# achinastone/Tensorium

Hardware: AMD Instinct MI355X
Metric: fp32 SGEMM GFLOP/s (M=N=K=4096) + YOLOv3 conv-fwd images/s (higher is better)
Workload: dtype fp32; 1 GPU; sgemm_nn_4096x4096x4096; M=4096, N=4096, K=4096, parallelism=1 independent replicas, one process per GPU, no data-path collective

## Files before the change

### tensorium_amd/csrc/sgemm_nn_big.hip

```cpp
#include <type_traits>

#include "tns_internal.hpp"

namespace tns {
namespace {

typedef float floatx16 __attribute__((ext_vector_type(16)));

template <int BM, int BN, int WM, int WN, int MINB, int BK = 32>
struct Geo {
  static constexpr int BM_ = BM, BN_ = BN, WN_ = WN, MINB_ = MINB, BK_ = BK;
  static constexpr int KQ = BK / 4;
  static constexpr int NT = 64 * WM * WN;
  static constexpr int WTM = BM / WM, WTN = BN / WN;
  static constexpr int TM = WTM / 32, TN = WTN / 32;
  static constexpr int LDA = BM, LDB = BN;
  static constexpr int A_TILE = BK * LDA, B_TILE = BK * LDB;
  static constexpr int STAGE = A_TILE + B_TILE;
  static constexpr int AU = BM * BK / 4 / NT;
  static constexpr int BROWS = 256 / BN;
  static constexpr int BDMA = BK / BROWS / (NT / 64);
  static_assert(TM == 2 || TM == 4, "A fragments read as one b64 / b128");
  static_assert(BN == 128 || BN == 256, "B rows of 512 B or 1 KB per DMA");
  static_assert(AU >= 1 && BDMA >= 1 && BM * BK / 4 % NT == 0, "staging split");
  static_assert(BK == 16 || BK == 32, "k-quad swizzle over at most 8 quads");
};

template <class G>
__global__ __launch_bounds__(G::NT, G::MINB_) void sgemm_nn_big_kernel(GemmArgs p) {
  constexpr int BM = G::BM_, BN = G::BN_, NT = G::NT, WN = G::WN_;
  constexpr int WTM = G::WTM, WTN = G::WTN, TM = G::TM, TN = G::TN;
  constexpr int LDA = G::LDA, LDB = G::LDB, A_TILE = G::A_TILE, STAGE = G::STAGE;
  constexpr int AU = G::AU, BK = G::BK_, KQ = G::KQ;
  constexpr int SW = KQ == 8 ? 2 : 4;
  const int tid = threadIdx.x, lane = tid & 63, wid = tid >> 6;
  const int lc = lane & 31, h = lane >> 5;
  const int wm = wid / WN, wn = wid % WN;
  __shared__ __attribute__((aligned(16))) float smem[2 * STAGE];

  const int tiles_m = (int)(p.M / BM), tiles_n = (int)(p.N / BN);
  int tm, tn;
  {
    const int nb = tiles_m * tiles_n, bid = blockIdx.x;
    const int xcd = bid & 7, q = nb >> 3, r = nb & 7;
    const int wg = (xcd < r ? xcd * (q + 1) : r * (q + 1) + (xcd - r) * q) + (bid >> 3);
    constexpr int GROUP_M = 8;
    const int per_group = GROUP_M * tiles_n;
    const int group = wg / per_group, first_m = group * GROUP_M;
    const int gsize = min(tiles_m - first_m, GROUP_M);
    const int in_group = wg - group * per_group;
    tm = first_m + in_group % gsize;
    tn = in_group / gsize;
  }
  const int64_t m0 = (int64_t)tm * BM, n0 = (int64_t)tn * BN, bz = blockIdx.y;
  const float* __restrict__ A = p.A + bz * p.strideA;
  const float* __restrict__ B = p.B + bz * p.strideB;
  float* __restrict__ C = p.C + bz * p.strideC;
  const int64_t lda = p.lda, ldb = p.ldb, ldc = p.ldc;

  floatx16 acc[TM][TN];
  const int64_t row_base = m0 + wm * WTM + 4 * h;
  const int64_t col_base = n0 + wn * WTN + lc;
  if (p.beta_mode == BETA_ZERO) {
#pragma unroll
    for (int i = 0; i < TM; ++i)
#pragma unroll
      for (int j = 0; j < TN; ++j)
#pragma unroll
        for (int e = 0; e < 16; ++e) acc[i][j][e] = 0.0f;
  } else {
    const bool scale = p.beta_mode == BETA_SCALE;
    const float beta = p.beta;
#pragma unroll
    for (int i = 0; i < TM; ++i)
#pragma unroll
      for (int j = 0; j < TN; ++j)
#pragma unroll
        for (int e = 0; e < 16; ++e)
          acc[i][j][e] = C[(row_base + 32 * i + (e & 3) + 8 * (e >> 2)) * ldc + col_base + 32 * j];
    if (scale) {
#pragma unroll
      for (int i = 0; i < TM; ++i)
#pragma unroll
        for (int j = 0; j < TN; ++j)
#pragma unroll
          for (int e = 0; e < 16; ++e) acc[i][j][e] = beta * acc[i][j][e];
    }
  }
#pragma unroll
  for (int i = 0; i < TM; ++i)
#pragma unroll
    for (int j = 0; j < TN; ++j) asm volatile("" : "+v"(acc[i][j]));

  const float* a_src[AU];
  int a_dst[AU];
#pragma unroll
  for (int u = 0; u < AU; ++u) {
    const int idx = tid + NT * u;
    const int kq = idx % KQ, mm = idx / KQ;
    const int m = (mm & ~(WTM - 1)) | ((mm % TM) << 5) | ((mm & (WTM - 1)) / TM);
    a_src[u] = A + (m0 + m) * lda + 4 * kq;
    a_dst[u] = (4 * kq) * LDA + (mm ^ (kq << SW));
  }
  float4 ra[AU];
  const float alpha = p.alpha;
  auto load_a = [&](int64_t k0) {
#pragma unroll
    for (int u = 0; u < AU; ++u) ra[u] = *reinterpret_cast<const float4*>(a_src[u] + k0);
  };
  auto store_a = [&](float* as) {
#pragma unroll
    for (int u = 0; u < AU; ++u) {
      float4 v = ra[u];
      v.x = alpha * v.x; v.y = alpha * v.y; v.z = alpha * v.z; v.w = alpha * v.w;
      as[a_dst[u]] = v.x;
      as[a_dst[u] + LDA] = v.y;
      as[a_dst[u] + 2 * LDA] = v.z;
      as[a_dst[u] + 3 * LDA] = v.w;
    }
  };
  constexpr int BROWS = G::BROWS, BDMA = G::BDMA;
  const int brow = BROWS * BDMA * wid + lane / (BN / 4);
  const float* b_src = B + (int64_t)brow * ldb + n0 + 4 * (lane % (BN / 4));
  const unsigned b_lds0 = __builtin_amdgcn_readfirstlane(
      (unsigned)(uintptr_t)(__attribute__((address_space(3))) float*)(smem + A_TILE +
                                                                      BROWS * BDMA * wid * LDB));
  auto dma_b = [&](int64_t k0, int stage) {
#pragma unroll
    for (int r = 0; r < BDMA; ++r) {
      unsigned keep;
      const float* src = b_src + (k0 + BROWS * r) * ldb;
      asm volatile(
          "s_mov_b32 %0, m0\n\ts_mov_b32 m0, %2\n\ts_nop 0\n\t"
          "global_load_lds_dwordx4 %1, off\n\ts_mov_b32 m0, %0"
          : "=&s"(keep)
          : "v"(src), "s"(b_lds0 + (unsigned)((stage * STAGE + BROWS * r * LDB) * 4))
          : "memory");
    }
  };

  const int a_frag = wm * WTM + TM * lc;
  const int b_frag = wn * WTN + lc;
  auto frag = [&](const float* st, int s, float (&a)[TM], float (&b)[TN]) {
    const int k = 2 * s + h;
#ifdef TNS_NB_NO_FRAG
    for (int i = 0; i < TM; ++i) a[i] = (float)(lane + i + s);
    for (int j = 0; j < TN; ++j) b[j] = (float)(lane - j + s);
    (void)st; (void)k;
    return;
#endif
    const float* ap = st + k * LDA + (a_frag ^ (((k >> 2) & (KQ - 1)) << SW));
    if constexpr (TM == 4) {
      const float4 v = *reinterpret_cast<const float4*>(ap);
      a[0] = v.x; a[1] = v.y; a[2] = v.z; a[3] = v.w;
    } else {
      const float2 v = *reinterpret_cast<const float2*>(ap);
      a[0] = v.x; a[1] = v.y;
    }
    const float* bp = st + A_TILE + k * LDB + b_frag;
#pragma unroll
    for (int j = 0; j < TN; ++j) b[j] = bp[32 * j];
  };
  auto mma = [&](const float (&a)[TM], const float (&b)[TN]) {
#pragma unroll
    for (int i = 0; i < TM; ++i)
#pragma unroll
      for (int j = 0; j < TN; ++j)
        acc[i][j] = __builtin_amdgcn_mfma_f32_32x32x2f32(a[i], b[j], acc[i][j], 0, 0, 0);
  };

  const int nt = (int)(p.K / BK);
  if (nt > 0) {
    load_a(0);
    dma_b(0, 0);
    store_a(smem);
    asm volatile("s_waitcnt vmcnt(0)" ::: "memory");
    __syncthreads();
  }
  auto tile = [&](int t, auto MORE) {
    constexpr bool more = decltype(MORE)::value;
    const float* cur = smem + (t & 1) * STAGE;
    float* nxt = smem + ((t + 1) & 1) * STAGE;
    if constexpr (more) {
#ifndef TNS_NB_NO_DMA
      dma_b((int64_t)(t + 1) * BK, (t + 1) & 1);
#endif
#ifndef TNS_NB_NO_AST
      load_a((int64_t)(t + 1) * BK);
#endif
      __builtin_amdgcn_sched_barrier(0);
    }
    float a0[TM], b0[TN], a1[TM], b1[TN];
    frag(cur, 0, a0, b0);
#pragma unroll
    for (int s = 0; s < BK / 2; s += 2) {
      frag(cur, s + 1, a1, b1);
      __builtin_amdgcn_sched_barrier(0);
      mma(a0, b0);
      if (s + 2 < BK / 2) frag(cur, s + 2, a0, b0);
      __builtin_amdgcn_sched_barrier(0);
      if constexpr (more)
        if (s == BK / 4 - 2) {
          __builtin_amdgcn_sched_barrier(0);
#ifndef TNS_NB_NO_AST
          store_a(nxt);
#endif
        }
      mma(a1, b1);
    }
    if constexpr (more) {
#ifndef TNS_NB_NO_BAR
      asm volatile("s_waitcnt vmcnt(0)" ::: "memory");
      __syncthreads();
#endif
    }
  };
  for (int t = 0; t + 1 < nt; ++t) tile(t, std::true_type{});
  if (nt > 0) tile(nt - 1, std::false_type{});

#pragma unroll
  for (int i = 0; i < TM; ++i)
#pragma unroll
    for (int e = 0; e < 16; ++e) {
      const int64_t row = row_base + 32 * i + (e & 3) + 8 * (e >> 2);
#pragma unroll
      for (int j = 0; j < TN; ++j) C[row * ldc + col_base + 32 * j] = acc[i][j][e];
    }
}

bool aligned16(const void* p) { return (reinterpret_cast<uintptr_t>(p) & 15) == 0; }

using G256 = Geo<256, 256, 2, 4, 1>;
using G128 = Geo<128, 128, 2, 2, 2>;
using G256x128 = Geo<256, 128, 2, 2, 1>;
using G256w16 = Geo<256, 256, 4, 4, 1>;
using G256x128k16 = Geo<256, 128, 2, 2, 2, 16>;

template <class G>
bool applies(const GemmArgs& a) {
  if (a.conv || a.epi != EPI_NONE || a.beta_mode == BETA_STORE) return false;
  if (a.M % G::BM_ || a.N % G::BN_ || a.K % G::BK_ || a.M <= 0 || a.N <= 0) return false;
  if (a.lda % 4 || a.ldb % 4 || !aligned16(a.A) || !aligned16(a.B)) return false;
  if (a.batch > 1 && (a.strideA % 4 || a.strideB % 4)) return false;
  return (a.M / G::BM_) * (a.N / G::BN_) <= 0x7fffffff;
}

template <class G>
hipError_t launch(const GemmArgs& a, hipStream_t s) {
  if (!applies<G>(a)) return hipErrorInvalidValue;
  const int64_t tiles = (a.M / G::BM_) * (a.N / G::BN_);
  for (int64_t b0 = 0; b0 < a.batch; b0 += 65535) {
    GemmArgs sub = a;
    const int64_t nb = a.batch - b0 < 65535 ? a.batch - b0 : 65535;
    sub.A = a.A + b0 * a.strideA;
    sub.B = a.B + b0 * a.strideB;
    sub.C = a.C + b0 * a.strideC;
    sub.batch = nb;
    hipLaunchKernelGGL(sgemm_nn_big_kernel<G>, dim3((unsigned)tiles, (unsigned)nb), dim3(G::NT), 0,
                       s, sub);
    hipError_t e = hipGetLastError();
    if (e != hipSuccess) return e;
  }
  return hipSuccess;
}

}

#ifdef TNS_DIAG_KERNELS
int sgemm_nn_big_count() { return 8; }
#else
int sgemm_nn_big_count() { return 7; }
#endif
const char* sgemm_nn_big_name(int v) {
  static const char* names[] = {"256x256x32_w2x4_nn_big", "128x128x32_w2x2_nn_big",
                                "256x128x32_w2x2_nn_big", "256x256x32_w4x4_nn_big",
                                "256x128x16_w2x2_b2_nn_big", "256x256x32_w2x4_pp_nn_big",
                                "256x256x32_w2x2_dma_nn_big", "256x256x32_w2x4_ppbq_nn_big"};
  return v >= 0 && v < sgemm_nn_big_count() ? names[v] : "";
}

int sgemm_nn_big_pick(const GemmArgs& a) {
  if (applies<G256>(a) && (a.M / 256) * (a.N / 256) * a.batch >= 192)
    return sgemm_nn_w4_applies(a) ? 6 : sgemm_nn_pp_applies(a) ? 5 : 0;
  return -1;
}

hipError_t launch_sgemm_nn_big(int v, const GemmArgs& a, hipStream_t s) {
  switch (v) {
    case 0: return launch<G256>(a, s);
    case 1: return launch<G128>(a, s);
    case 2: return launch<G256x128>(a, s);
    case 3: return launch<G256w16>(a, s);
    case 4: return launch<G256x128k16>(a, s);
    case 5: return launch_sgemm_nn_pp(a, s);
    case 6: return launch_sgemm_nn_w4(a, s);
#ifdef TNS_DIAG_KERNELS
    case 7: return launch_sgemm_nn_pp(a, s, true);
#endif
    default: return hipErrorInvalidValue;
  }
}

}
```

### tensorium_amd/csrc/sgemm_nn_w4.hip

```cpp
#include "tns_internal.hpp"

namespace tns {
namespace {

typedef float floatx16 __attribute__((ext_vector_type(16)));
typedef float floatx4 __attribute__((ext_vector_type(4)));
typedef int int4v __attribute__((ext_vector_type(4)));

constexpr int BM = 256, BN = 256, BK = 32, NT = 256;
constexpr int A_TILE = BM * BK, B_TILE = BK * BN, STAGE = A_TILE + B_TILE;

__device__ __forceinline__ void dma16(const float* sbase, unsigned voff, unsigned lds) {
  unsigned keep;
  asm volatile(
      "s_mov_b32 %0, m0\n\ts_mov_b32 m0, %3\n\ts_nop 0\n\t"
      "global_load_lds_dwordx4 %1, %2\n\ts_mov_b32 m0, %0"
      : "=&s"(keep)
      : "v"(voff), "s"(sbase), "s"(lds)
      : "memory");
}

template <bool ALPHA1>
__global__ __launch_bounds__(NT, 1) void sgemm_nn_w4_kernel(GemmArgs p) {
  __shared__ __attribute__((aligned(16))) float smem[2 * STAGE];
  const int tid = threadIdx.x, lane = tid & 63;
  const int wid = __builtin_amdgcn_readfirstlane(tid >> 6);
  const int lc = lane & 31, h = lane >> 5;
  const int wm = wid >> 1, wn = wid & 1;

  const int tiles_m = (int)(p.M / BM), tiles_n = (int)(p.N / BN);
  int tm, tn;
  const int64_t bz = blockIdx.y;
  {
    const int nb = tiles_m * tiles_n, bid = blockIdx.x;
    const int xcd = bid & 7, q = nb >> 3, r = nb & 7;
    const int wg = (xcd < r ? xcd * (q + 1) : r * (q + 1) + (xcd - r) * q) + (bid >> 3);
    constexpr int GROUP_M = 8;
    const int per_group = GROUP_M * tiles_n;
    const int group = wg / per_group, first_m = group * GROUP_M;
    const int gsize = min(tiles_m - first_m, GROUP_M);
    const int in_group = wg - group * per_group;
    tm = first_m + in_group % gsize;
    tn = in_group / gsize;
  }
  const int64_t m0 = (int64_t)tm * BM, n0 = (int64_t)tn * BN;
  const float* __restrict__ A = p.A + bz * p.strideA;
  const float* __restrict__ B = p.B + bz * p.strideB;
  float* __restrict__ C = p.C + bz * p.strideC;
  const int64_t lda = p.lda, ldb = p.ldb, ldc = p.ldc;

  const int arow = lane >> 3;
  const unsigned a_voff = (unsigned)(arow * lda * 4) + 16u * (unsigned)((lane & 7) ^ ((arow >> 1) & 7));
  const unsigned a_voff1 = (unsigned)(arow * lda * 4) +
                           16u * (unsigned)((lane & 7) ^ (((arow >> 1) & 7) ^ 4));
  const unsigned b_voff0 = 16u * (unsigned)lane;
  const unsigned b_voff1 = 16u * (unsigned)((lane + 8) & 63);
  const unsigned lds0 = (unsigned)(uintptr_t)(__attribute__((address_space(3))) float*)smem;
  const float* a_row0 = A + m0 * lda;
  const float* b_row0 = B + n0;
  auto issue1 = [&](int u, int64_t k0, int st) {
    const unsigned sb = lds0 + (unsigned)(st * STAGE * 4);
    if (u < 8) {
      const int q = 8 * wid + u;
      dma16(a_row0 + (int64_t)(8 * q) * lda + k0, (u & 1) ? a_voff1 : a_voff,
            sb + (unsigned)(q * 1024));
    } else {
      const int r = 8 * wid + (u - 8);
      dma16(b_row0 + (k0 + r) * ldb, (u & 1) ? b_voff1 : b_voff0,
            sb + (unsigned)(A_TILE * 4 + r * 1024));
    }
  };
  auto issue = [&](int64_t k0, int st) {
    const unsigned sb = lds0 + (unsigned)(st * STAGE * 4);
#pragma unroll
    for (int u = 0; u < 8; ++u) {
      const int q = 8 * wid + u;
      dma16(a_row0 + (int64_t)(8 * q) * lda + k0, (u & 1) ? a_voff1 : a_voff,
            sb + (unsigned)(q * 1024));
    }
#pragma unroll
    for (int u = 0; u < 8; ++u) {
      const int r = 8 * wid + u;
      dma16(b_row0 + (k0 + r) * ldb, (u & 1) ? b_voff1 : b_voff0,
            sb + (unsigned)(A_TILE * 4 + r * 1024));
    }
  };

  const int nt = (int)(p.K / BK);
#ifdef TNS_W4_DMA_LATE
  constexpr bool kDmaFirst = false;
#else
  constexpr bool kDmaFirst = true;
#endif
  if (kDmaFirst && nt > 0) issue(0, 0);
  if (kDmaFirst && nt > 1) issue(BK, 1);

  floatx16 acc[4][4];
  const int64_t row_base = m0 + wm * 128;
  const __amdgpu_buffer_rsrc_t crs = __builtin_amdgcn_make_buffer_rsrc(
      C + row_base * ldc, 0, 0x7fffffff, 0x00020000);
  const unsigned c_voff = 4u * (unsigned)(4 * h * ldc + n0 + wn * 128 + 4 * lc);
  auto c_soff = [&](int i, int e) {
    return (unsigned)(4 * (32 * i + (e & 3) + 8 * (e >> 2)) * ldc);
  };
  if (p.beta_mode == BETA_ZERO) {
#pragma unroll
    for (int i = 0; i < 4; ++i)
#pragma unroll
      for (int j = 0; j < 4; ++j)
#pragma unroll
        for (int e = 0; e < 16; ++e) acc[i][j][e] = 0.0f;
  } else {
    const bool scale = p.beta_mode == BETA_SCALE;
    const float beta = p.beta;
    {
      floatx4 v[2][4];
      auto ldv = [&](int g, floatx4 (&t)[4]) {
#pragma unroll
        for (int u = 0; u < 4; ++u)
          t[u] = __builtin_bit_cast(floatx4, __builtin_amdgcn_raw_buffer_load_b128(
                                                 crs, c_voff, c_soff(g >> 2, 4 * (g & 3) + u), 0));
      };
      ldv(0, v[0]);
#pragma unroll
      for (int g = 0; g < 16; ++g) {
        if (g + 1 < 16) ldv(g + 1, v[(g + 1) & 1]);
#pragma unroll
        for (int u = 0; u < 4; ++u)
#pragma unroll
          for (int j = 0; j < 4; ++j) {
            const float c = v[g & 1][u][j];
            acc[g >> 2][j][4 * (g & 3) + u] = scale ? beta * c : c;
          }
      }
    }
  }
#pragma unroll
  for (int i = 0; i < 4; ++i)
#pragma unroll
    for (int j = 0; j < 4; ++j) asm volatile("" : "+a"(acc[i][j]));
  if (!kDmaFirst && nt > 0) issue(0, 0);
  if (!kDmaFirst && nt > 1) issue(BK, 1);

  const int swz = (lc >> 1) & 7;
  int b_col[4];
#pragma unroll
  for (int j = 0; j < 4; ++j)
    b_col[j] = A_TILE + h * BN + ((wn * 128 + 4 * lc + j - 32 * h) & 255);
  const float alpha = p.alpha;
  auto mma = [&](const float (&a)[4], const float (&b)[4]) {
    float aa[4];
#pragma unroll
    for (int i = 0; i < 4; ++i) aa[i] = ALPHA1 ? a[i] : alpha * a[i];
#pragma unroll
    for (int i = 0; i < 4; ++i)
#pragma unroll
      for (int j = 0; j < 4; ++j)
        acc[i][j] = __builtin_amdgcn_mfma_f32_32x32x2f32(aa[i], b[j], acc[i][j], 0, 0, 0);
  };
  auto mma_dma = [&](const float (&a)[4], const float (&b)[4], int64_t k0, int st, bool dma) {
    float aa[4];
#pragma unroll
    for (int i = 0; i < 4; ++i) aa[i] = ALPHA1 ? a[i] : alpha * a[i];
#pragma unroll
    for (int u = 0; u < 16; ++u) {
      const int i = u >> 2, j = u & 3;
      acc[i][j] = __builtin_amdgcn_mfma_f32_32x32x2f32(aa[i], b[j], acc[i][j], 0, 0, 0);
      if (dma) issue1(u, k0, st);
      __builtin_amdgcn_sched_barrier(0);
    }
  };

  const int a_lane = (wm * 128 + lc) * BK + h;
  auto frag = [&](const float* st, int s, float (&a)[4], float (&b)[4]) {
    const int ka = 4 * ((s >> 1) ^ swz) + 2 * (s & 1);
#pragma unroll
    for (int i = 0; i < 4; ++i) a[i] = st[a_lane + 32 * BK * i + ka];
    const floatx4 v = *reinterpret_cast<const floatx4*>(st + b_col[0] + 2 * s * BN);
    b[0] = v[0]; b[1] = v[1]; b[2] = v[2]; b[3] = v[3];
  };
  float a0[4], b0[4], a1[4], b1[4];
  {
    if (nt > 0) {
      if (nt > 1) {
        asm volatile("s_waitcnt vmcnt(16)" ::: "memory");
      } else {
        asm volatile("s_waitcnt vmcnt(0)" ::: "memory");
      }
      __syncthreads();
      frag(smem, 0, a0, b0);
    }
    for (int t = 0; t < nt; ++t) {
      const float* cur = smem + (t & 1) * STAGE;
      const float* nxt = smem + ((t + 1) & 1) * STAGE;
#pragma unroll
      for (int s = 0; s < BK / 2 - 2; s += 2) {
        frag(cur, s + 1, a1, b1);
        __builtin_amdgcn_sched_barrier(0);
        mma(a0, b0);
        frag(cur, s + 2, a0, b0);
        __builtin_amdgcn_sched_barrier(0);
        mma(a1, b1);
      }
      frag(cur, BK / 2 - 1, a1, b1);
      __builtin_amdgcn_sched_barrier(0);
      mma(a0, b0);
      __builtin_amdgcn_sched_barrier(0);
      if (t + 1 < nt) {
        asm volatile("s_waitcnt vmcnt(0)" ::: "memory");
        __syncthreads();
        frag(nxt, 0, a0, b0);
        __builtin_amdgcn_sched_barrier(0);
      }
      mma_dma(a1, b1, (int64_t)(t + 2) * BK, t & 1, t + 2 < nt);
    }
  }

#pragma unroll
  for (int i = 0; i < 4; ++i)
#pragma unroll
    for (int e = 0; e < 16; ++e) {
      const floatx4 v = {acc[i][0][e], acc[i][1][e], acc[i][2][e], acc[i][3][e]};
      __builtin_amdgcn_raw_buffer_store_b128(__builtin_bit_cast(int4v, v), crs, c_voff,
                                             c_soff(i, e), 0);
    }
}

bool aligned16(const void* q) { return (reinterpret_cast<uintptr_t>(q) & 15) == 0; }

}

bool sgemm_nn_w4_applies(const GemmArgs& a) {
  if (a.conv || a.epi != EPI_NONE || a.beta_mode == BETA_STORE) return false;
  if (a.M % BM || a.N % BN || a.K % BK || a.M <= 0 || a.N <= 0) return false;
  if (a.lda % 4 || a.ldb % 4 || !aligned16(a.A) || !aligned16(a.B)) return false;
  if (a.batch > 1 && (a.strideA % 4 || a.strideB % 4)) return false;
  if (a.lda * 4 * 8 > 0x7fffffffLL || (256 * a.ldc + a.N) * 4 > 0x7fffffffLL) return false;
  return (a.M / BM) * (a.N / BN) <= 0x7fffffff;
}

hipError_t launch_sgemm_nn_w4(const GemmArgs& a, hipStream_t s) {
  if (!sgemm_nn_w4_applies(a)) return hipErrorInvalidValue;
  const int64_t tiles = (a.M / BM) * (a.N / BN);
  const bool alpha1 = a.alpha == 1.0f;
  for (int64_t b0 = 0; b0 < a.batch; b0 += 65535) {
    GemmArgs sub = a;
    const int64_t nb = a.batch - b0 < 65535 ? a.batch - b0 : 65535;
    sub.A = a.A + b0 * a.strideA;
    sub.B = a.B + b0 * a.strideB;
    sub.C = a.C + b0 * a.strideC;
    sub.batch = nb;
    const dim3 grid((unsigned)tiles, (unsigned)nb);
    if (alpha1)
      hipLaunchKernelGGL((sgemm_nn_w4_kernel<true>), grid, dim3(NT), 0, s, sub);
    else
      hipLaunchKernelGGL((sgemm_nn_w4_kernel<false>), grid, dim3(NT), 0, s, sub);
    hipError_t e = hipGetLastError();
    if (e != hipSuccess) return e;
  }
  return hipSuccess;
}

}
```

### tensorium_amd/csrc/tns_internal.hpp

```cpp
#pragma once
#include <hip/hip_runtime.h>
#include <stdint.h>

#include "../../include/tns.h"

namespace tns {

int set_error(int code, const char* fmt, ...);
const char* hip_err_str(hipError_t e);

#define TNS_HIP_TRY(expr)                                                              \
  do {                                                                                 \
    hipError_t _e = (expr);                                                            \
    if (_e != hipSuccess)                                                              \
      return ::tns::set_error(TNS_ERR_HIP, "%s failed: %s (%s:%d)", #expr,            \
                              ::tns::hip_err_str(_e), __FILE__, __LINE__);             \
  } while (0)

enum EpiKind { EPI_NONE = 0, EPI_BIAS_ACT = 1, EPI_ADD = 2 };
constexpr bool act_transcendental(int act) { return act == 0 || act == 6; }

enum BetaMode { BETA_ZERO = 0, BETA_ONE = 1, BETA_SCALE = 2, BETA_STORE = 3 };

struct GemmArgs {
  int64_t M, N, K;
  float alpha, beta;
  int beta_mode;
  const float* A;
  int64_t lda, strideA;
  const float* B;
  int64_t ldb, strideB;
  float* C;
  int64_t ldc, strideC;
  int64_t batch;
  int epi;
  const float* bias;
  int act;
  int conv;
  const int* ktab;
  int ktab_n;
  int conv_H, conv_W, conv_ow, conv_ohw, conv_sY, conv_sX, conv_pH, conv_pW;
  int conv_bytes;
  int dx_cls, dx_taps, dx_imgW;
  unsigned* stamps;
};

hipError_t launch_sgemm(const GemmArgs& a, bool transA, bool transB, hipStream_t s);
int sgemm_nn_big_count();
const char* sgemm_nn_big_name(int v);
int sgemm_nn_big_pick(const GemmArgs& a);
hipError_t launch_sgemm_nn_big(int v, const GemmArgs& a, hipStream_t s);
bool sgemm_nn_pp_applies(const GemmArgs& a);
hipError_t launch_sgemm_nn_pp(const GemmArgs& a, hipStream_t s, bool bperm = false);
bool sgemm_nn_w4_applies(const GemmArgs& a);
hipError_t launch_sgemm_nn_w4(const GemmArgs& a, hipStream_t s);
hipError_t launch_sgemm_nt_sdot(const GemmArgs& a, hipStream_t s);
hipError_t launch_sdot_chains(const GemmArgs& a, int variant, hipStream_t s);
int sdot_chains_variant_count();
const char* sdot_chains_variant_name(int v);
int sdot_rc_variant_count();
const char* sdot_rc_variant_name(int v);
bool sdot_rc_applies(const GemmArgs& a);
hipError_t launch_sdot_rc(int v, const GemmArgs& a, hipStream_t s);
constexpr int SDOT_FORM_RC = 64;
void set_sdot_form(int form);
hipError_t launch_sgemm_tt(const GemmArgs& a, hipStream_t s);
hipError_t launch_add_in_order(float* C, const float* part, int64_t n, int64_t batch,
                               hipStream_t s);
hipError_t launch_sgemm_conv(const GemmArgs& a, hipStream_t s);
hipError_t launch_sgemm_conv_variant(int variant, const GemmArgs& a, hipStream_t s);
int conv_tile_count();
const char* conv_tile_name(int v);
int conv_tile_pick(const GemmArgs& a, int ks);
hipError_t launch_conv_tile(int v, const GemmArgs& a, int ks, int dil, hipStream_t s);
struct ConvSlabArgs {
  const float* input;
  const float* weights;
  const float* bias;
  float* out;
  int64_t batch, C, H, W, M, K, ks, stride, pad, dil, ow, ohw;
  int act;
};
int conv1x1_count();
const char* conv1x1_name(int v);
int conv1x1_pick(int64_t M, int64_t N, int64_t K, int64_t P);
hipError_t launch_conv1x1(int v, const float* weights, const float* x, const float* bias,
                          float* out, int64_t batch, int64_t M, int64_t K, int64_t P, int act,
                          hipStream_t s, bool add = false);
hipError_t launch_transpose(const float* in, float* out, int64_t rows, int64_t cols,
                            hipStream_t s);
int conv_slab_count();
const char* conv_slab_name(int v);
int conv_slab_pick(int64_t M, int64_t N, int64_t K, int64_t ks);
int64_t conv_slab_floats(int v, int64_t N, int64_t K);
hipError_t launch_conv_slab(int v, const ConvSlabArgs& c, float* slab, hipStream_t s);
int conv_tile4_count();
bool conv_tile4_is_ap(int v);
bool conv_tile_is_ap(int v);
hipError_t conv_tile4_permute(const float* A, float* Ap, int64_t M, int64_t K, hipStream_t s);
const char* conv_tile4_name(int v);
int conv_tile4_bk(int v);
hipError_t launch_conv_tile4(int v, const GemmArgs& a, int ks, int dil, hipStream_t s);
int conv_tile4_ta_count();
const char* conv_tile4_ta_name(int v);
int conv_tile4_dx_pick(int64_t M, int64_t N, int64_t K, int64_t ks);
hipError_t launch_conv_tile4_dx(int v, const float* w, const float* delta, float* col,
                                int64_t batch, int64_t C, int64_t ks, int64_t F, int64_t oh,
                                int64_t ow, hipStream_t s, bool add_into = false);
int conv_tile4_dx3_count();
const char* conv_tile4_dx3_name(int v);
int conv_tile4_dx3_pick(int64_t batch, int64_t C, int64_t H, int64_t W, int64_t F, int64_t ks,
                        int64_t pad);
hipError_t launch_conv_tile4_dx3(int v, const float* wt, const float* delta, float* im,
                                 int64_t batch, int64_t C, int64_t H, int64_t W, int64_t F,
                                 int64_t ks, int64_t pad, int64_t oh, int64_t ow, hipStream_t s);
hipError_t launch_transpose_taps(const float* w, float* wt, int64_t F, int64_t C, int64_t K2,
                                 hipStream_t s, unsigned long long order = ~0ULL);
unsigned long long conv_tile4_dx3s2_order(int64_t pad);
int conv_tile4_dx3s2_pick(int64_t batch, int64_t C, int64_t H, int64_t W, int64_t F, int64_t ks,
                          int64_t pad);
hipError_t launch_conv_tile4_dx3s2(int v, const float* wt, const float* delta, float* im,
                                   int64_t batch, int64_t C, int64_t H, int64_t W, int64_t F,
                                   int64_t pad, int64_t oh, int64_t ow, hipStream_t s);
int conv_pp_count();
const char* conv_pp_name(int v);
int conv_pp_pick(const GemmArgs& a, int ks);
hipError_t launch_conv_pp(int v, const GemmArgs& a, int ks, int dil, hipStream_t s);
int conv_dma_count();
const char* conv_dma_name(int v);
int conv_dma_pick(const GemmArgs& a, int ks);
hipError_t launch_conv_dma(int v, const GemmArgs& a, int ks, int dil, hipStream_t s);
int conv_patch_count();
const char* conv_patch_name(int v);
int conv_patch_pick(const GemmArgs& a);
hipError_t launch_conv_patch(int v, const GemmArgs& a, hipStream_t s);
struct DwArgs {
  const float* delta;
  const float* x;
  float* part;
  int M, N, HW, C, H, W, oW, stride, pad, dil;
  int va;
  float alpha;
  int64_t strideA, strideX, strideP, batch;
};
int dw_tile_count();
const char* dw_tile_name(int v);
int dw_tile_pick(const DwArgs& a, int ks);
hipError_t launch_dw_tile(int v, const DwArgs& a, int ks, hipStream_t s);
bool conv_direct_applies(int64_t C, int64_t ks, int64_t filters);
hipError_t launch_conv_direct(const float* in, const float* w, const float* bias, float* out,
                              int64_t batch, int64_t C, int64_t H, int64_t W, int64_t filters,
                              int64_t ks, int64_t stride, int64_t pad, int64_t dil, int64_t oh,
                              int64_t ow, int act, hipStream_t s);
bool conv_dx_fused_applies(int64_t C, int64_t H, int64_t W, int64_t ks, int64_t stride, int64_t F,
                           int64_t oh, int64_t ow);
bool conv_dx_fused_fits(int64_t C, int64_t H, int64_t W, int64_t stride, int64_t F, int64_t oh,
                        int64_t ow);
hipError_t launch_conv_dx_col2im(const float* w, float* wt, const float* delta, float* im,
                                 int64_t batch, int64_t C, int64_t H, int64_t W, int64_t F,
                                 int64_t ks, int64_t pad, int64_t dil, int64_t oh, int64_t ow,
                                 hipStream_t s);
constexpr int KTAB_PAD = 256;
hipError_t launch_build_ktab(int* ktab, int C, int Hs, int Ws, int kH, int kW, int dY, int dX,
                             hipStream_t s);
hipError_t launch_pad_images(const float* im, int64_t batch, int64_t C, int64_t H, int64_t W,
                             int64_t pH, int64_t pW, float* out, hipStream_t s);
hipError_t launch_sgemm_variant(int variant, const GemmArgs& a, bool transA, bool transB,
                                hipStream_t s);
int sgemm_variant_count();
const char* sgemm_variant_name(int v);

struct ConvGeom {
  int64_t C, H, W, kH, kW, padH, padW, sY, sX, dY, dX;
  int64_t oh, ow;
};
int64_t out_dim(int64_t in, int64_t pad, int64_t k, int64_t dil, int64_t stride);
hipError_t launch_im2col(const ConvGeom& g, const float* im, int64_t imStride, float* col,
                         int64_t colStride, int64_t batch, hipStream_t s);
hipError_t launch_col2im(const ConvGeom& g, const float* col, int64_t colStride, float* im,
                         int64_t imStride, int64_t batch, hipStream_t s);
struct DwResArgs {
  ConvGeom g;
  const float* x;
  int64_t xStride;
  const float* delta;
  float* weight_updates;
  float *dA, *dB, *part;
  int64_t M, N, K, batch;
  bool direct;
  float alpha;
};
int dw_res_count();
const char* dw_res_name(int v);
int64_t dw_res_k4(int64_t K);
int64_t dw_res_groups(int v);
int64_t dw_res_b_rows(int v, int64_t N);
int dw_res_pick(int64_t M, int64_t N, int64_t K, int64_t batch);
hipError_t launch_dw_res(int v, const DwResArgs& d, hipStream_t s);

bool act_supported(int act);
hipError_t launch_forward_bias(float* dst, int64_t nFilters, int64_t blockSize,
                               const float* bias, int64_t incb, int64_t batch, hipStream_t s);
hipError_t launch_backward_bias(float* dst, int64_t nDst, const float* src, int64_t blockSize,
                                int64_t batch, int64_t incb, hipStream_t s);
hipError_t launch_activate(float* x, int64_t n, int act, hipStream_t s);
hipError_t launch_shortcut(int64_t n, const float* a, const float* b, float* out, int act,
                           hipStream_t s);
hipError_t launch_upsample(int64_t planes, int H, int W, int stride, float scale, const float* in,
                           float* out, hipStream_t s);
hipError_t launch_upsample_backward(int64_t planes, int H, int W, int stride, float scale,
                                   float* in, const float* out, int zero, hipStream_t s);
struct PoolGeom {
  int h, w, outH, outW, size, sx, sy, off;
};
hipError_t launch_maxpool_forward(int64_t planes, const PoolGeom& g, const float* in, float* out,
                                  int64_t* indexes, hipStream_t s);
hipError_t launch_avgpool_forward(int64_t planes, const PoolGeom& g, const float* in, float* out,
                                  hipStream_t s);
hipError_t launch_maxpool_backward(int64_t planes, const PoolGeom& g, float* state_delta,
                                   const int64_t* indexes, const float* delta, hipStream_t s);
hipError_t launch_avgpool_backward(int64_t planes, const PoolGeom& g, float* state_delta,
                                   const float* delta, hipStream_t s);
hipError_t launch_dropout_forward(int64_t n, uint32_t seed, float probability, float scale,
                                  const float* src, float* rnd, float* dst, hipStream_t s);
hipError_t launch_dropout_backward(int64_t n, float probability, float scale, const float* src,
                                   const float* rnd, float* dst, hipStream_t s);
hipError_t launch_cost_l2(int64_t n, const float* pred, const float* truth, float* delta,
                          float* error, hipStream_t s);
hipError_t launch_xent_logistic(int64_t n, const float* pred, const float* truth, float* delta,
                                float* error, hipStream_t s);
hipError_t launch_lstm_gates_forward(int64_t n, const float* const w[4], const float* const u[4],
                                     float* c_state, float* h_state, float* cell_slice,
                                     float* out_slice, hipStream_t s);
hipError_t launch_lstm_gates_backward(int64_t n, const float* const w[4], const float* const u[4],
                                      const float* cell_i, const float* cprev,
                                      const float* delta_i, float* dc, float* const dw[4],
                                      float* const du[4], hipStream_t s);
hipError_t launch_vv(int op, int64_t n, const float* a, int64_t inca, const float* b, int64_t incb,
                     const float* c, int64_t incc, float* d, int64_t incd, hipStream_t s);
hipError_t launch_fmavss(int64_t n, const float* src, float scalar, float bias, float* dst,
                         hipStream_t s);
hipError_t launch_inverse_sqrt(int64_t n, const float* src, float* dst, int64_t stride,
                               hipStream_t s);
hipError_t launch_yolo(int64_t batch, int anchors, int classes, int64_t hw, const float* in,
                       float* out, hipStream_t s);
hipError_t launch_bias_activate(float* dst, int64_t nFilters, int64_t blockSize,
                                const float* bias, int64_t batch, int act, hipStream_t s);
hipError_t launch_derive(const float* x, int64_t n, int act, float* delta, hipStream_t s);
hipError_t launch_sgd_update(int64_t nw, float* w, float* dw, int64_t n, float* b, float* db,
                             float* sc, float* dsc, float lrb, float ndb, float mom,
                             hipStream_t s);
hipError_t launch_axpy(int64_t n, float a, const float* x, int64_t incx, float* y, int64_t incy,
                       hipStream_t s);
hipError_t launch_scale(int64_t n, float a, float* x, int64_t stride, hipStream_t s);
hipError_t launch_fill(int64_t n, float* x, float v, int64_t stride, hipStream_t s);
hipError_t launch_copy(int64_t n, const float* src, int64_t inca, float* dst, int64_t incb,
                       hipStream_t s);
hipError_t launch_clamp(int64_t n, float alpha, const float* src, float* dst, int64_t stride,
                        hipStream_t s);

hipError_t launch_means_vars(const float* x, int64_t groups, int64_t N, int64_t bs, float* means,
                             float* vars, int quirk, float* part, hipStream_t s, int what = 3);
hipError_t launch_normalize(float* x, int64_t groups, int64_t N, int64_t bs, const float* means,
                            int64_t mstride, const float* vars, int64_t vstride, hipStream_t s);
hipError_t launch_scale_add(float* x, int64_t groups, int64_t N, int64_t bs, const float* scales,
                            const float* biases, int64_t incb, hipStream_t s);
hipError_t launch_add_dots(float* dst, const float* a, const float* b, int64_t groups, int64_t N,
                           int64_t bs, float* part, hipStream_t s);
hipError_t launch_add_sums(float* dst, const float* src, int64_t groups, int64_t N, int64_t bs,
                           float* part, hipStream_t s);
hipError_t launch_derive_add_sums(float* dst, float* delta, const float* output, int act,
                                  int64_t groups, int64_t N, int64_t bs, float* part,
                                  hipStream_t s);
hipError_t launch_mean_var_delta(const float* delta, const float* x, const float* mean,
                                 const float* var, int64_t groups, int64_t N, int64_t bs,
                                 float* mean_delta, float* var_delta, int quirk, float* part,
                                 hipStream_t s, const float* scales = nullptr);
hipError_t launch_normalize_delta(const float* x, const float* mean, const float* var,
                                  const float* mean_delta, const float* var_delta, float* delta,
                                  int64_t groups, int64_t N, int64_t bs, hipStream_t s, const float* scales = nullptr); 
bool bn_folds_scale(int64_t bs);
hipError_t launch_bn_backward_fused(float* scale_updates, const float* x_norm, float* delta,
                                    const float* output, int act, const float* x,
                                    const float* mean, const float* var, const float* scales,
                                    float* mean_delta, float* var_delta, int64_t groups,
                                    int64_t N, int64_t bs, int quirk, float* part, hipStream_t s);
hipError_t launch_add_dots_derive(float* dst, const float* x_norm, float* delta,
                                  const float* output, int act, int64_t groups, int64_t N,
                                  int64_t bs, float* part, hipStream_t s);
hipError_t launch_bn_apply(const float* y, float* x, float* xn, float* out, int64_t groups,
                           int64_t N, int64_t bs, const float* means, const float* vars,
                           const float* scales, const float* biases, int act, hipStream_t s);
hipError_t launch_rolling_update(int64_t n, float* rm, float* rv, const float* mean,
                                 const float* var, float momentum, hipStream_t s);
hipError_t launch_softmax_batch(int64_t n, const float* in, int64_t batch, int64_t batch_size,
                                int64_t groups, int64_t group_size, int64_t stride, float temp,
                                float* out, hipStream_t s);
hipError_t launch_xent_softmax(int64_t n, const float* pred, const float* truth, float* delta,
                               float* error, hipStream_t s);
hipError_t launch_vssum(int64_t n, const float* a, float* out, hipStream_t s);

constexpr int MLP_MAX_LAYERS = 16;
struct MlpArgs {
  int nlayers;
  int64_t widths[MLP_MAX_LAYERS + 1];
  int acts[MLP_MAX_LAYERS];
  int bn;
  int64_t batch;
  const float* X;
  const float* truth;
  float lr, momentum, decay;
  float* buf;
  float* cost;
  int64_t off[MLP_MAX_LAYERS][16];
  int64_t softmax_off;
  int64_t stamp_off;
  int lds_chunks;
  int64_t act_off;
  float* l0part;
};
int64_t mlp_buffer_floats(int nlayers, const int64_t* widths, int bn, int64_t batch);
hipError_t launch_mlp_train_step(const MlpArgs& a, hipStream_t s);

}
```

Before: 143,900 GFLOP/s.

## Add row-wise prologue/epilogue to w4 SGEMM overlapping C load/store with MFMA

Adds a ROWS variant of the w4 kernel, the new default, that splits the prologue and epilogue into per-accumulator-row units. It streams C loads (beta path) and C stores row by row underneath the first and last K tiles' MFMAs instead of doing them all before or after the main loop. The aim is to hide the C read and write latency at the tile boundaries. It adds considerable code complexity, hand-written inline asm buffer loads, and a new dependence on correct waitcnt accounting.

Measured after the change: 146,500 GFLOP/s, median of 6. 1.8% higher.

```diff
diff --git a/tensorium_amd/csrc/sgemm_nn_big.hip b/tensorium_amd/csrc/sgemm_nn_big.hip
--- a/tensorium_amd/csrc/sgemm_nn_big.hip
+++ b/tensorium_amd/csrc/sgemm_nn_big.hip
@@ -267,15 +267,16 @@
 }
 
 #ifdef TNS_DIAG_KERNELS
+int sgemm_nn_big_count() { return 9; }
+#else
 int sgemm_nn_big_count() { return 8; }
-#else
-int sgemm_nn_big_count() { return 7; }
 #endif
 const char* sgemm_nn_big_name(int v) {
   static const char* names[] = {"256x256x32_w2x4_nn_big", "128x128x32_w2x2_nn_big",
                                 "256x128x32_w2x2_nn_big", "256x256x32_w4x4_nn_big",
                                 "256x128x16_w2x2_b2_nn_big", "256x256x32_w2x4_pp_nn_big",
-                                "256x256x32_w2x2_dma_nn_big", "256x256x32_w2x4_ppbq_nn_big"};
+                                "256x256x32_w2x2_dma_nn_big", "256x256x32_w2x2_dma_flat_nn_big",
+                                "256x256x32_w2x4_ppbq_nn_big"};
   return v >= 0 && v < sgemm_nn_big_count() ? names[v] : "";
 }
 
@@ -293,9 +294,10 @@
     case 3: return launch<G256w16>(a, s);
     case 4: return launch<G256x128k16>(a, s);
     case 5: return launch_sgemm_nn_pp(a, s);
-    case 6: return launch_sgemm_nn_w4(a, s);
+    case 6: return launch_sgemm_nn_w4(a, s, true);
+    case 7: return launch_sgemm_nn_w4(a, s, false);
 #ifdef TNS_DIAG_KERNELS
-    case 7: return launch_sgemm_nn_pp(a, s, true);
+    case 8: return launch_sgemm_nn_pp(a, s, true);
 #endif
     default: return hipErrorInvalidValue;
   }
diff --git a/tensorium_amd/csrc/sgemm_nn_w4.hip b/tensorium_amd/csrc/sgemm_nn_w4.hip
--- a/tensorium_amd/csrc/sgemm_nn_w4.hip
+++ b/tensorium_amd/csrc/sgemm_nn_w4.hip
@@ -1,3 +1,5 @@
+#include <type_traits>
+
 #include "tns_internal.hpp"
 
 namespace tns {
@@ -9,6 +11,7 @@
 
 constexpr int BM = 256, BN = 256, BK = 32, NT = 256;
 constexpr int A_TILE = BM * BK, B_TILE = BK * BN, STAGE = A_TILE + B_TILE;
+constexpr int ROWS_MIN_TILES = 4;
 
 __device__ __forceinline__ void dma16(const float* sbase, unsigned voff, unsigned lds) {
   unsigned keep;
@@ -20,9 +23,21 @@
       : "memory");
 }
 
-template <bool ALPHA1>
+#ifdef TNS_W4_STAMPS
+#define TNS_W4_STAMP(i) stamp[i] = __builtin_amdgcn_s_memtime()
+#else
+#define TNS_W4_STAMP(i) \
+  do {                  \
+  } while (0)
+#endif
+
+template <bool ALPHA1, bool ROWS>
 __global__ __launch_bounds__(NT, 1) void sgemm_nn_w4_kernel(GemmArgs p) {
   __shared__ __attribute__((aligned(16))) float smem[2 * STAGE];
+#ifdef TNS_W4_STAMPS
+  unsigned long long stamp[4];
+  TNS_W4_STAMP(0);
+#endif
   const int tid = threadIdx.x, lane = tid & 63;
   const int wid = __builtin_amdgcn_readfirstlane(tid >> 6);
   const int lc = lane & 31, h = lane >> 5;
@@ -87,13 +102,6 @@
   };
 
   const int nt = (int)(p.K / BK);
-#ifdef TNS_W4_DMA_LATE
-  constexpr bool kDmaFirst = false;
-#else
-  constexpr bool kDmaFirst = true;
-#endif
-  if (kDmaFirst && nt > 0) issue(0, 0);
-  if (kDmaFirst && nt > 1) issue(BK, 1);
 
   floatx16 acc[4][4];
   const int64_t row_base = m0 + wm * 128;
@@ -103,44 +111,6 @@
   auto c_soff = [&](int i, int e) {
     return (unsigned)(4 * (32 * i + (e & 3) + 8 * (e >> 2)) * ldc);
   };
-  if (p.beta_mode == BETA_ZERO) {
-#pragma unroll
-    for (int i = 0; i < 4; ++i)
-#pragma unroll
-      for (int j = 0; j < 4; ++j)
-#pragma unroll
-        for (int e = 0; e < 16; ++e) acc[i][j][e] = 0.0f;
-  } else {
-    const bool scale = p.beta_mode == BETA_SCALE;
-    const float beta = p.beta;
-    {
-      floatx4 v[2][4];
-      auto ldv = [&](int g, floatx4 (&t)[4]) {
-#pragma unroll
-        for (int u = 0; u < 4; ++u)
-          t[u] = __builtin_bit_cast(floatx4, __builtin_amdgcn_raw_buffer_load_b128(
-                                                 crs, c_voff, c_soff(g >> 2, 4 * (g & 3) + u), 0));
-      };
-      ldv(0, v[0]);
-#pragma unroll
-      for (int g = 0; g < 16; ++g) {
-        if (g + 1 < 16) ldv(g + 1, v[(g + 1) & 1]);
-#pragma unroll
-        for (int u = 0; u < 4; ++u)
-#pragma unroll
-          for (int j = 0; j < 4; ++j) {
-            const float c = v[g & 1][u][j];
-            acc[g >> 2][j][4 * (g & 3) + u] = scale ? beta * c : c;
-          }
-      }
-    }
-  }
-#pragma unroll
-  for (int i = 0; i < 4; ++i)
-#pragma unroll
-    for (int j = 0; j < 4; ++j) asm volatile("" : "+a"(acc[i][j]));
-  if (!kDmaFirst && nt > 0) issue(0, 0);
-  if (!kDmaFirst && nt > 1) issue(BK, 1);
 
   const int swz = (lc >> 1) & 7;
   int b_col[4];
@@ -180,7 +150,79 @@
     b[0] = v[0]; b[1] = v[1]; b[2] = v[2]; b[3] = v[3];
   };
   float a0[4], b0[4], a1[4], b1[4];
-  {
+  auto flat_tile = [&](int t, bool pub, bool dma) {
+    const float* cur = smem + (t & 1) * STAGE;
+    const float* nxt = smem + ((t + 1) & 1) * STAGE;
+#pragma unroll
+    for (int s = 0; s < BK / 2 - 2; s += 2) {
+      frag(cur, s + 1, a1, b1);
+      __builtin_amdgcn_sched_barrier(0);
+      mma(a0, b0);
+      frag(cur, s + 2, a0, b0);
+      __builtin_amdgcn_sched_barrier(0);
+      mma(a1, b1);
+    }
+    frag(cur, BK / 2 - 1, a1, b1);
+    __builtin_amdgcn_sched_barrier(0);
+    mma(a0, b0);
+    __builtin_amdgcn_sched_barrier(0);
+    if (pub) {
+      asm volatile("s_waitcnt vmcnt(0)" ::: "memory");
+      __syncthreads();
+      frag(nxt, 0, a0, b0);
+      __builtin_amdgcn_sched_barrier(0);
+    }
+    mma_dma(a1, b1, (int64_t)(t + 2) * BK, t & 1, dma);
+  };
+
+  if constexpr (!ROWS) {
+#ifdef TNS_W4_DMA_LATE
+    constexpr bool kDmaFirst = false;
+#else
+    constexpr bool kDmaFirst = true;
+#endif
+    if (kDmaFirst && nt > 0) issue(0, 0);
+    if (kDmaFirst && nt > 1) issue(BK, 1);
+
+    if (p.beta_mode == BETA_ZERO) {
+#pragma unroll
+      for (int i = 0; i < 4; ++i)
+#pragma unroll
+        for (int j = 0; j < 4; ++j)
+#pragma unroll
+          for (int e = 0; e < 16; ++e) acc[i][j][e] = 0.0f;
+    } else {
+      const bool scale = p.beta_mode == BETA_SCALE;
+      const float beta = p.beta;
+      {
+        floatx4 v[2][4];
+        auto ldv = [&](int g, floatx4 (&t)[4]) {
+#pragma unroll
+          for (int u = 0; u < 4; ++u)
+            t[u] = __builtin_bit_cast(floatx4, __builtin_amdgcn_raw_buffer_load_b128(
+                                                   crs, c_voff, c_soff(g >> 2, 4 * (g & 3) + u), 0));
+        };
+        ldv(0, v[0]);
+#pragma unroll
+        for (int g = 0; g < 16; ++g) {
+          if (g + 1 < 16) ldv(g + 1, v[(g + 1) & 1]);
+#pragma unroll
+          for (int u = 0; u < 4; ++u)
+#pragma unroll
+            for (int j = 0; j < 4; ++j) {
+              const float c = v[g & 1][u][j];
+              acc[g >> 2][j][4 * (g & 3) + u] = scale ? beta * c : c;
+            }
+        }
+      }
+    }
+#pragma unroll
+    for (int i = 0; i < 4; ++i)
+#pragma unroll
+      for (int j = 0; j < 4; ++j) asm volatile("" : "+a"(acc[i][j]));
+    if (!kDmaFirst && nt > 0) issue(0, 0);
+    if (!kDmaFirst && nt > 1) issue(BK, 1);
+
     if (nt > 0) {
       if (nt > 1) {
         asm volatile("s_waitcnt vmcnt(16)" ::: "memory");
@@ -190,43 +232,234 @@
       __syncthreads();
       frag(smem, 0, a0, b0);
     }
-    for (int t = 0; t < nt; ++t) {
-      const float* cur = smem + (t & 1) * STAGE;
-      const float* nxt = smem + ((t + 1) & 1) * STAGE;
+    TNS_W4_STAMP(1);
+    for (int t = 0; t < nt; ++t) flat_tile(t, t + 1 < nt, t + 2 < nt);
+    TNS_W4_STAMP(2);
+
+#pragma unroll
+    for (int i = 0; i < 4; ++i)
+#pragma unroll
+      for (int e = 0; e < 16; ++e) {
+        const floatx4 v = {acc[i][0][e], acc[i][1][e], acc[i][2][e], acc[i][3][e]};
+        __builtin_amdgcn_raw_buffer_store_b128(__builtin_bit_cast(int4v, v), crs, c_voff,
+                                               c_soff(i, e), 0);
+      }
+  } else {
+    float fa0, fa1, fb0[4], fb1[4];
+    auto rfrag = [&](const float* st, int s, int i, float& a, float (&b)[4]) {
+      const int ka = 4 * ((s >> 1) ^ swz) + 2 * (s & 1);
+      a = st[a_lane + 32 * BK * i + ka];
+      const floatx4 v = *reinterpret_cast<const floatx4*>(st + b_col[0] + 2 * s * BN);
+      b[0] = v[0]; b[1] = v[1]; b[2] = v[2]; b[3] = v[3];
+    };
+    auto rmma = [&](auto I_, float a, const float (&b)[4]) {
+      constexpr int I = decltype(I_)::value;
+      const float aa = ALPHA1 ? a : alpha * a;
+#pragma unroll
+      for (int j = 0; j < 4; ++j)
+        acc[I][j] = __builtin_amdgcn_mfma_f32_32x32x2f32(aa, b[j], acc[I][j], 0, 0, 0);
+    };
+    auto bar = [&]() { asm volatile("s_waitcnt lgkmcnt(0)\n\ts_barrier" ::: "memory"); };
+    auto none = [] {};
+    auto none1 = [](int) {};
+    using R0 = std::integral_constant<int, 0>;
+    using R1 = std::integral_constant<int, 1>;
+    using R2 = std::integral_constant<int, 2>;
+    using R3 = std::integral_constant<int, 3>;
+    using RN = std::integral_constant<int, -1>;
+    auto unit = [&](auto I_, const float* st, auto NI_, const float* nst, auto&& mid,
+                    auto&& after) {
+      constexpr int I = decltype(I_)::value, NI = decltype(NI_)::value;
 #pragma unroll
       for (int s = 0; s < BK / 2 - 2; s += 2) {
-        frag(cur, s + 1, a1, b1);
+        rfrag(st, s + 1, I, fa1, fb1);
         __builtin_amdgcn_sched_barrier(0);
-        mma(a0, b0);
-        frag(cur, s + 2, a0, b0);
+        rmma(I_, fa0, fb0);
+        after(s);
+        rfrag(st, s + 2, I, fa0, fb0);
         __builtin_amdgcn_sched_barrier(0);
-        mma(a1, b1);
+        rmma(I_, fa1, fb1);
+        after(s + 1);
       }
-      frag(cur, BK / 2 - 1, a1, b1);
-      __builtin_amdgcn_sched_barrier(0);
-      mma(a0, b0);
-      __builtin_amdgcn_sched_barrier(0);
-      if (t + 1 < nt) {
-        asm volatile("s_waitcnt vmcnt(0)" ::: "memory");
-        __syncthreads();
-        frag(nxt, 0, a0, b0);
+      rfrag(st, BK / 2 - 1, I, fa1, fb1);
+      __builtin_amdgcn_sched_barrier(0);
+      rmma(I_, fa0, fb0);
+      after(BK / 2 - 2);
+      __builtin_amdgcn_sched_barrier(0);
+      mid();
+      if constexpr (NI >= 0) {
+        rfrag(nst, 0, NI, fa0, fb0);
         __builtin_amdgcn_sched_barrier(0);
       }
-      mma_dma(a1, b1, (int64_t)(t + 2) * BK, t & 1, t + 2 < nt);
-    }
+      rmma(I_, fa1, fb1);
+      after(BK / 2 - 1);
+      __builtin_amdgcn_sched_barrier(0);
+    };
+    const float* const S0 = smem;
+    const float* const S1 = smem + STAGE;
+
+    int tb;
+    if (p.beta_mode == BETA_ZERO) {
+      issue(0, 0);
+      issue(BK, 1);
+#pragma unroll
+      for (int i = 0; i < 4; ++i)
+#pragma unroll
+        for (int j = 0; j < 4; ++j) {
+#pragma unroll
+          for (int e = 0; e < 16; ++e) acc[i][j][e] = 0.0f;
+          asm volatile("" : "+a"(acc[i][j]));
+        }
+      asm volatile("s_waitcnt vmcnt(16)" ::: "memory");
+      bar();
+      TNS_W4_STAMP(1);
+      tb = 0;
+    } else {
+      const bool scale = p.beta_mode == BETA_SCALE;
+      const float beta = p.beta;
+      const uint64_t cb = (uint64_t)(uintptr_t)(C + row_base * ldc);
+      const int4v crs_raw = {(int)(uint32_t)cb, (int)((uint32_t)(cb >> 32) & 0xffffu), 0x7fffffff,
+                             0x00020000};
+      floatx4 va[16], vb[16];
+      auto ldrow = [&](int i, floatx4 (&v)[16]) {
+#pragma unroll
+        for (int e = 0; e < 16; ++e) {
+          const unsigned so = c_soff(i, e);
+          if (e == 0)
+            asm volatile("s_nop 4\n\tbuffer_load_dwordx4 %0, %1, %2, %3 offen"
+                         : "=&v"(v[e])
+                         : "v"(c_voff), "s"(crs_raw), "s"(so)
+                         : "memory");
+          else
+            asm volatile("buffer_load_dwordx4 %0, %1, %2, %3 offen"
+                         : "=&v"(v[e])
+                         : "v"(c_voff), "s"(crs_raw), "s"(so)
+                         : "memory");
+        }
+      };
+      auto waitrow = [&](auto N_, floatx4 (&v)[16]) {
+        asm volatile("s_waitcnt vmcnt(%[n])"
+                     : "+v"(v[0]), "+v"(v[1]), "+v"(v[2]), "+v"(v[3]), "+v"(v[4]), "+v"(v[5]),
+                       "+v"(v[6]), "+v"(v[7])
+                     : [n] "n"(decltype(N_)::value)
+                     : "memory");
+        asm volatile(""
+                     : "+v"(v[8]), "+v"(v[9]), "+v"(v[10]), "+v"(v[11]), "+v"(v[12]), "+v"(v[13]),
+                       "+v"(v[14]), "+v"(v[15])
+                     :
+                     : "memory");
+      };
+      auto mvrow = [&](auto I_, const floatx4 (&v)[16]) {
+        constexpr int I = decltype(I_)::value;
+#pragma unroll
+        for (int j = 0; j < 4; ++j) {
+#pragma unroll
+          for (int e = 0; e < 16; ++e) {
+            const float c = v[e][j];
+            acc[I][j][e] = scale ? beta * c : c;
+          }
+          asm volatile("" : "+a"(acc[I][j]));
+        }
+      };
+      using N0 = std::integral_constant<int, 0>;
+      using N16 = std::integral_constant<int, 16>;
+      using N32 = std::integral_constant<int, 32>;
+
+      issue(0, 0);
+      ldrow(0, va);
+      issue(BK, 1);
+      ldrow(1, vb);
+      waitrow(N32{}, va);
+      bar();
+      mvrow(R0{}, va);
+      ldrow(2, va);
+      rfrag(S0, 0, 0, fa0, fb0);
+      __builtin_amdgcn_sched_barrier(0);
+      TNS_W4_STAMP(1);
+      unit(R0{}, S0, R0{}, S1, [&] {
+        asm volatile("s_waitcnt vmcnt(32)" ::: "memory");
+        bar();
+      }, none1);
+      unit(R0{}, S1, R1{}, S0, [&] {
+        waitrow(N16{}, vb);
+        mvrow(R1{}, vb);
+        ldrow(3, vb);
+      }, none1);
+      unit(R1{}, S0, R1{}, S1, none, none1);
+      unit(R1{}, S1, R2{}, S0, [&] {
+        waitrow(N16{}, va);
+        mvrow(R2{}, va);
+      }, none1);
+      unit(R2{}, S0, R3{}, S0, [&] {
+        waitrow(N0{}, vb);
+        mvrow(R3{}, vb);
+      }, none1);
+      unit(R3{}, S0, R2{}, S1, none, none1);
+      bar();
+      unit(R2{}, S1, R3{}, S1, none, [&](int s) {
+        if (s < 8) {
+          issue1(2 * s, 2 * BK, 0);
+          issue1(2 * s + 1, 2 * BK, 0);
+        }
+      });
+      unit(R3{}, S1, RN{}, S1, none, none1);
+      asm volatile("s_waitcnt vmcnt(0)" ::: "memory");
+      bar();
+      issue(3 * BK, 1);
+      tb = 2;
+    }
+
+    const float* const sA = smem + (nt & 1) * STAGE;
+    const float* const sB = smem + ((nt + 1) & 1) * STAGE;
+    if (tb < nt - 2) {
+      frag(S0, 0, a0, b0);
+      for (int t = tb; t < nt - 2; ++t) flat_tile(t, true, true);
+      fa0 = a0[0];
+#pragma unroll
+      for (int j = 0; j < 4; ++j) fb0[j] = b0[j];
+    } else {
+      rfrag(sA, 0, 0, fa0, fb0);
+    }
+    __builtin_amdgcn_sched_barrier(0);
+
+    auto store1 = [&](auto I_, int e) {
+      constexpr int I = decltype(I_)::value;
+      const floatx4 v = {acc[I][0][e], acc[I][1][e], acc[I][2][e], acc[I][3][e]};
+      __builtin_amdgcn_raw_buffer_store_b128(__builtin_bit_cast(int4v, v), crs, c_voff,
+                                             c_soff(I, e), 0);
+    };
+    unit(R0{}, sA, R1{}, sA, none, none1);
+    unit(R1{}, sA, R0{}, sB, [&] {
+      asm volatile("s_waitcnt vmcnt(0)" ::: "memory");
+      bar();
+    }, none1);
+    unit(R0{}, sB, R1{}, sB, none, none1);
+    unit(R1{}, sB, R2{}, sA, none, [&](int s) { store1(R0{}, s); });
+    unit(R2{}, sA, R2{}, sB, none, [&](int s) { store1(R1{}, s); });
+    unit(R2{}, sB, R3{}, sA, none, none1);
+    unit(R3{}, sA, R3{}, sB, none, [&](int s) { store1(R2{}, s); });
+    unit(R3{}, sB, RN{}, sB, none, none1);
+    TNS_W4_STAMP(2);
+#pragma unroll
+    for (int e = 0; e < 16; ++e) store1(R3{}, e);
   }
-
-#pragma unroll
-  for (int i = 0; i < 4; ++i)
-#pragma unroll
-    for (int e = 0; e < 16; ++e) {
-      const floatx4 v = {acc[i][0][e], acc[i][1][e], acc[i][2][e], acc[i][3][e]};
-      __builtin_amdgcn_raw_buffer_store_b128(__builtin_bit_cast(int4v, v), crs, c_voff,
-                                             c_soff(i, e), 0);
-    }
+#ifdef TNS_W4_STAMPS
+  asm volatile("s_waitcnt vmcnt(0)" ::: "memory");
+  TNS_W4_STAMP(3);
+  const unsigned blk = blockIdx.y * gridDim.x + blockIdx.x;
+  if (lane == 0 && p.stamps != nullptr && blk < (1u << 16)) {
+    unsigned long long* d = reinterpret_cast<unsigned long long*>(p.stamps) + (4 * blk + wid) * 4;
+#pragma unroll
+    for (int i = 0; i < 4; ++i) d[i] = stamp[i];
+  }
+#endif
 }
 
 bool aligned16(const void* q) { return (reinterpret_cast<uintptr_t>(q) & 15) == 0; }
+
+#ifdef TNS_W4_STAMPS
+unsigned* g_w4_stamps = nullptr;
+#endif
 
 }
 
@@ -239,10 +472,11 @@
   return (a.M / BM) * (a.N / BN) <= 0x7fffffff;
 }
 
-hipError_t launch_sgemm_nn_w4(const GemmArgs& a, hipStream_t s) {
+hipError_t launch_sgemm_nn_w4(const GemmArgs& a, hipStream_t s, bool rows) {
   if (!sgemm_nn_w4_applies(a)) return hipErrorInvalidValue;
   const int64_t tiles = (a.M / BM) * (a.N / BN);
   const bool alpha1 = a.alpha == 1.0f;
+  rows = rows && a.K / BK >= ROWS_MIN_TILES;
   for (int64_t b0 = 0; b0 < a.batch; b0 += 65535) {
     GemmArgs sub = a;
     const int64_t nb = a.batch - b0 < 65535 ? a.batch - b0 : 65535;
@@ -250,15 +484,29 @@
     sub.B = a.B + b0 * a.strideB;
     sub.C = a.C + b0 * a.strideC;
     sub.batch = nb;
+#ifdef TNS_W4_STAMPS
+    sub.stamps = g_w4_stamps;
+#endif
     const dim3 grid((unsigned)tiles, (unsigned)nb);
-    if (alpha1)
-      hipLaunchKernelGGL((sgemm_nn_w4_kernel<true>), grid, dim3(NT), 0, s, sub);
+    if (rows && alpha1)
+      hipLaunchKernelGGL((sgemm_nn_w4_kernel<true, true>), grid, dim3(NT), 0, s, sub);
+    else if (rows)
+      hipLaunchKernelGGL((sgemm_nn_w4_kernel<false, true>), grid, dim3(NT), 0, s, sub);
+    else if (alpha1)
+      hipLaunchKernelGGL((sgemm_nn_w4_kernel<true, false>), grid, dim3(NT), 0, s, sub);
     else
-      hipLaunchKernelGGL((sgemm_nn_w4_kernel<false>), grid, dim3(NT), 0, s, sub);
+      hipLaunchKernelGGL((sgemm_nn_w4_kernel<false, false>), grid, dim3(NT), 0, s, sub);
     hipError_t e = hipGetLastError();
     if (e != hipSuccess) return e;
   }
   return hipSuccess;
 }
 
-}
+#ifdef TNS_W4_STAMPS
+extern "C" int tns_debug_w4_stamps(unsigned* dev_buf) {
+  g_w4_stamps = dev_buf;
+  return 0;
+}
+#endif
+
+}
diff --git a/tensorium_amd/csrc/tns_internal.hpp b/tensorium_amd/csrc/tns_internal.hpp
--- a/tensorium_amd/csrc/tns_internal.hpp
+++ b/tensorium_amd/csrc/tns_internal.hpp
@@ -53,7 +53,7 @@
 bool sgemm_nn_pp_applies(const GemmArgs& a);
 hipError_t launch_sgemm_nn_pp(const GemmArgs& a, hipStream_t s, bool bperm = false);
 bool sgemm_nn_w4_applies(const GemmArgs& a);
-hipError_t launch_sgemm_nn_w4(const GemmArgs& a, hipStream_t s);
+hipError_t launch_sgemm_nn_w4(const GemmArgs& a, hipStream_t s, bool rows = true);
 hipError_t launch_sgemm_nt_sdot(const GemmArgs& a, hipStream_t s);
 hipError_t launch_sdot_chains(const GemmArgs& a, int variant, hipStream_t s);
 int sdot_chains_variant_count();
```
